# clairesonglee/HierarchicalGNN

Hardware: AMD Instinct MI355X
Metric: edges aggregated/sec on TrackML-1GeV graphs, latent=256 (higher is better)
Workload: dtype f32

## Files before the change

### hierarchicalgnn_amd/build.py

```python
from __future__ import annotations

import glob
import os
import shutil
import subprocess
import sys

HERE = os.path.dirname(os.path.abspath(__file__))
CSRC = os.path.join(HERE, "csrc")
OUT = os.path.join(CSRC, "libhgnn_hip.so")
ARCH = "gfx950"


def sources():
    return sorted(glob.glob(os.path.join(CSRC, "*.hip")))


def _deps():
    return sources() + sorted(glob.glob(os.path.join(CSRC, "*.h"))) + \
        [os.path.join(HERE, "..", "include", "hgnn_hip.h")]


def up_to_date() -> bool:
    if not os.path.exists(OUT):
        return False
    t = os.path.getmtime(OUT)
    return all(os.path.getmtime(p) <= t for p in _deps())


def build(force: bool = False, verbose: bool = True) -> str:
    if not force and up_to_date():
        return OUT
    hipcc = shutil.which("hipcc") or "/opt/rocm/bin/hipcc"
    if not os.path.exists(hipcc):
        raise RuntimeError("hipcc not found: cannot build libhgnn_hip.so")
    objs = []
    procs = []
    for src in sources():
        obj = src[:-4] + ".o"
        objs.append(obj)
        if not force and os.path.exists(obj) and all(
                os.path.getmtime(p) <= os.path.getmtime(obj)
                for p in [src] + [d for d in _deps() if d.endswith(".h")]):
            continue
        cmd = [hipcc, "-O3", "-std=c++17", f"--offload-arch={ARCH}", "-fPIC", "-c", src, "-o", obj]
        if verbose:
            print(" ".join(cmd), flush=True)
        procs.append((cmd, subprocess.Popen(cmd)))
    for cmd, p in procs:
        if p.wait() != 0:
            raise RuntimeError("build failed: " + " ".join(cmd))
    cmd = [hipcc, f"--offload-arch={ARCH}", "-shared", "-fPIC", "-o", OUT] + objs
    if verbose:
        print(" ".join(cmd), flush=True)
    subprocess.check_call(cmd)
    return OUT


if __name__ == "__main__":
    print(build(force="--force" in sys.argv))
```

### hierarchicalgnn_amd/csrc/capi.hip

```cpp
#include "common.h"
#include "options.h"
#include <climits>
#include <cstdlib>
#include <cstring>

namespace hgnn {
static thread_local char g_err[512] = "";

void set_error(const char* fmt, ...) {
    va_list ap;
    va_start(ap, fmt);
    vsnprintf(g_err, sizeof(g_err), fmt, ap);
    va_end(ap);
}

static const struct {
    const char* name;
    int* value;
    int lo, hi;
    const char* takes;
} kOptions[] = {
    {"nt_loads", &g_opt_nt_loads, INT_MIN, INT_MAX, nullptr},
    {"nt_stores", &g_opt_nt_stores, INT_MIN, INT_MAX, nullptr},
    {"k1_one_launch", &g_opt_k1_one_launch, 0, 1, "takes 0 or 1"},
    {"k1_item_order", &g_opt_k1_item_order, 0, 1, "takes 0 or 1"},
#ifdef HGNN_K1_SWEEP
    {"k1_window", &g_opt_k1_window, INT_MIN, INT_MAX, nullptr},
    {"k1_waves", &g_opt_k1_waves, INT_MIN, INT_MAX, nullptr},
#endif
    {"mlp_ablate", &g_opt_mlp_ablate, INT_MIN, INT_MAX, nullptr},
    {"mlp_split_variant", &g_opt_mlp_split_variant, INT_MIN, INT_MAX, nullptr},
    {"mlp_split3_rows128", &f3::g_opt_split3_rows128, 0, 2,
     "takes 0 or 1 (2 = experimental tile, needs HGNN_EXPERIMENTAL=1)"},
    {"mlp_split3_one_wg", &f3::g_opt_split3_one_wg, INT_MIN, INT_MAX, nullptr},
};
}

using namespace hgnn;

extern "C" int hgnn_abi_version(void) { return HGNN_ABI_VERSION; }
extern "C" const char* hgnn_last_error(void) { return hgnn::g_err; }
extern "C" int hgnn_sizeof_plan(void) { return (int)sizeof(hgnn_plan); }
extern "C" int hgnn_sizeof_mlp_desc(void) { return (int)sizeof(hgnn_mlp_desc); }

extern "C" int hgnn_set_option(const char* name, int value) {
    HGNN_REQUIRE(name != nullptr, "hgnn_set_option: name is NULL");
    for (const auto& o : kOptions) {
        if (strcmp(name, o.name)) continue;
        const bool experimental = o.value == &f3::g_opt_split3_rows128 && value == 2;
        if (value < o.lo || value > o.hi || (experimental && getenv("HGNN_EXPERIMENTAL") == nullptr)) {
            set_error("hgnn_set_option: %s %s", o.name, o.takes);
            return HGNN_ERR_INVALID_ARG;
        }
        *o.value = o.value == &g_opt_mlp_ablate ? value & 31 : value;
        return HGNN_OK;
    }
    set_error("hgnn_set_option: unknown option '%s'", name);
    return HGNN_ERR_INVALID_ARG;
}

extern "C" int hgnn_get_option(const char* name, int* value) {
    HGNN_REQUIRE(name != nullptr && value != nullptr, "hgnn_get_option: NULL pointer");
    for (const auto& o : kOptions) {
        if (strcmp(name, o.name)) continue;
        *value = *o.value;
        return HGNN_OK;
    }
    set_error("hgnn_get_option: unknown option '%s'", name);
    return HGNN_ERR_INVALID_ARG;
}
```

### hierarchicalgnn_amd/csrc/options.h

```cpp
#pragma once

namespace hgnn {

extern int g_opt_nt_loads;
extern int g_opt_nt_stores;
extern int g_opt_k1_one_launch;
extern int g_opt_k1_item_order;
#ifdef HGNN_K1_SWEEP
extern int g_opt_k1_window;
extern int g_opt_k1_waves;
#endif
extern int g_opt_mlp_ablate;
extern int g_opt_mlp_split_variant;
namespace f3 {
extern int g_opt_split3_rows128;
extern int g_opt_split3_one_wg;
}

}
```

### hierarchicalgnn_amd/csrc/rows_common.h

```cpp
#pragma once
#include "common.h"
#include "options.h"
#include <type_traits>

namespace hgnn {

typedef float f32x4 __attribute__((ext_vector_type(4)));

struct ItemView {
    const int32_t *begin, *end, *target;
    const int32_t* n_items;
    int64_t max_items;
    const int32_t *src_row, *perm, *wi_dst;
};

static inline ItemView work_items(const hgnn_plan* p) {
    return {p->wi_begin, p->wi_end, p->wi_target, p->counts + HGNN_CNT_WORK, p->max_work,
            p->src_row, p->perm, p->wi_dst};
}

static inline ItemView split_items(const hgnn_plan* p) {
    return {p->split_pbegin, p->split_pbegin + 1, p->split_dst, p->counts + HGNN_CNT_SPLIT, p->max_split,
            nullptr, nullptr, nullptr};
}

struct ItemExtra {
    const int32_t* order;
    int32_t* arrive;
    const int32_t *split_pbegin, *split_dst, *n_split;
    int32_t max_split;
};

static inline ItemExtra item_extra(const hgnn_plan* p, const int32_t* order, int32_t* arrive) {
    return {order, arrive, p->split_pbegin, p->split_dst, p->counts + HGNN_CNT_SPLIT, (int32_t)p->max_split};
}

template <int MAX_COLS, class Fn>
static inline void for_row_shape(int ncol, Fn&& fn) {
    using std::integral_constant;
    constexpr integral_constant<int, 1> one{};
    if (ncol <= 4) fn(integral_constant<int, 4>{}, one);
    else if (ncol <= 8) fn(integral_constant<int, 8>{}, one);
    else if (ncol <= 16) fn(integral_constant<int, 16>{}, one);
    else if (ncol <= 32) fn(integral_constant<int, 32>{}, one);
    else if (MAX_COLS <= 64 || ncol <= 64) fn(integral_constant<int, 64>{}, one);
    else if constexpr (MAX_COLS > 64) {
        if (ncol <= 128) fn(integral_constant<int, 64>{}, integral_constant<int, 2>{});
        else fn(integral_constant<int, 64>{}, integral_constant<int, 4>{});
    }
}

template <int WPB, class... P, class... A>
static inline void launch_items(void (*kernel)(P...), int64_t max_items, hipStream_t s, A... args) {
    const unsigned grid = (unsigned)ceil_div(max_items, WPB);
    if (grid) kernel<<<grid, WPB * 64, 0, s>>>(args...);
}

static inline unsigned capped_grid(int64_t blocks) {
    const int64_t cap = 256 * 8 * 4;
    return (unsigned)(blocks < 1 ? 1 : blocks > cap ? cap : blocks);
}
static inline unsigned stream_grid(int64_t n_tiles) { return capped_grid(ceil_div(n_tiles, kWavesPerBlock)); }

}
```

### hierarchicalgnn_amd/csrc/segreduce.hip

```cpp
#include "rows_common.h"

namespace hgnn {

int g_opt_nt_loads = 1;
int g_opt_nt_stores = 0;
int g_opt_k1_one_launch = 1;
int g_opt_k1_item_order = 0;

template <bool NT>
__device__ __forceinline__ f32x4 ld4(const void* p) {
    if constexpr (NT) return __builtin_nontemporal_load((const f32x4*)p);
    else return *(const f32x4*)p;
}

__device__ __forceinline__ bool last_chunk_arrives(const ItemExtra& x, int p, int lane, int& pbegin, int& nch,
                                                   int& dst) {
    int s = 0, hi = min(*x.n_split, x.max_split);
    while (hi - s > 1) {
        const int mid = (s + hi) >> 1;
        if (x.split_pbegin[mid] <= p) s = mid;
        else hi = mid;
    }
    pbegin = x.split_pbegin[s];
    nch = x.split_pbegin[s + 1] - pbegin;
    dst = x.split_dst[s];
    asm volatile("s_waitcnt vmcnt(0)" ::: "memory");
    __builtin_amdgcn_fence(__ATOMIC_RELEASE, "agent");
    asm volatile("s_waitcnt vmcnt(0)" ::: "memory");
    int seen = 0;
    if (lane == 0) seen = __hip_atomic_fetch_add(&x.arrive[s], 1, __ATOMIC_ACQ_REL, __HIP_MEMORY_SCOPE_AGENT);
    if (__builtin_amdgcn_readfirstlane(seen) != nch - 1) return false;
    asm volatile("s_waitcnt vmcnt(0)" ::: "memory");
    if (lane == 0) __hip_atomic_store(&x.arrive[s], 0, __ATOMIC_RELAXED, __HIP_MEMORY_SCOPE_AGENT);
    return true;
}

template <int RL, int VPL, int U, bool HAS_W, bool HAS_RS, bool NT, int TAG, int WPB, bool XCD>
__global__ __launch_bounds__(WPB * 64) void k_seg_reduce(
    const float* __restrict__ src, int F, int nvec, const int32_t* __restrict__ src_row,
    const int32_t* __restrict__ perm, const float* __restrict__ weight,
    const float* __restrict__ row_scale, const int32_t* __restrict__ wi_begin,
    const int32_t* __restrict__ wi_end, const int32_t* __restrict__ wi_target,
    const int32_t* __restrict__ n_items_ptr, int64_t max_items, float* __restrict__ out,
    float* __restrict__ partial, ItemExtra x) {
    constexpr int G = 64 / RL;
    const int lane = threadIdx.x & 63;
    int64_t bid = blockIdx.x;
    if (XCD) {
        const int64_t per_xcd = (gridDim.x + 7) / 8;
        bid = (bid % 8) * per_xcd + bid / 8;
    }
    int64_t item = bid * WPB + (threadIdx.x >> 6);
    const int n_items = *n_items_ptr;
    if (item >= max_items) return;
    if (x.order != nullptr) item = x.order[item];
    if (item >= n_items || item >= max_items) return;
    const int begin = __builtin_amdgcn_readfirstlane(wi_begin[item]);
    const int end = __builtin_amdgcn_readfirstlane(wi_end[item]);
    const int target = __builtin_amdgcn_readfirstlane(wi_target[item]);
    const int g = lane / RL;
    const int c = lane % RL;

    f32x4 acc[VPL];
#pragma unroll
    for (int v = 0; v < VPL; ++v) acc[v] = f32x4{0.f, 0.f, 0.f, 0.f};

    for (int base = begin; base < end; base += 64) {
        const int n = (end - base) < 64 ? (end - base) : 64;
        int my_row = 0;
        float my_w = 1.f;
        if (lane < n) {
            const int p = base + lane;
            my_row = src_row != nullptr ? src_row[p] : p;
            if (HAS_W) my_w = weight[perm != nullptr ? perm[p] : p];
            if (HAS_RS) my_w *= row_scale[my_row];
        }
        for (int j = 0; j < n; j += G * U) {
            f32x4 val[U][VPL];
            float w[U];
#pragma unroll
            for (int u = 0; u < U; ++u) {
                const int e = j + u * G + g;
                int r;
                if (G == 1) {
                    r = __builtin_amdgcn_readlane(my_row, (j + u) & 63);
                    w[u] = (HAS_W || HAS_RS)
                               ? __builtin_bit_cast(float, __builtin_amdgcn_readlane(
                                                               __builtin_bit_cast(int, my_w), (j + u) & 63))
                               : 1.f;
                } else {
                    r = __shfl(my_row, e & 63);
                    w[u] = (HAS_W || HAS_RS) ? __shfl(my_w, e & 63) : 1.f;
                }
                const bool ok = e < n;
                const float* rp = src + (size_t)r * (size_t)F;
#pragma unroll
                for (int v = 0; v < VPL; ++v) {
                    const int cv = c + v * 64;
                    if (ok && cv < nvec)
                        val[u][v] = ld4<NT>(rp + cv * 4);
                    else
                        val[u][v] = f32x4{0.f, 0.f, 0.f, 0.f};
                }
            }
#pragma unroll
            for (int u = 0; u < U; ++u) {
#pragma unroll
                for (int v = 0; v < VPL; ++v) {
                    if (HAS_W || HAS_RS)
                        acc[v] += val[u][v] * w[u];
                    else
                        acc[v] += val[u][v];
                }
            }
        }
    }
    if (G > 1) {
#pragma unroll
        for (int off = RL; off < 64; off <<= 1) {
#pragma unroll
            for (int v = 0; v < VPL; ++v) {
                acc[v].x += __shfl_xor(acc[v].x, off);
                acc[v].y += __shfl_xor(acc[v].y, off);
                acc[v].z += __shfl_xor(acc[v].z, off);
                acc[v].w += __shfl_xor(acc[v].w, off);
            }
        }
    }
    if (g == 0) {
        float* op = target >= 0 ? out + (size_t)target * (size_t)F
                                : partial + (size_t)(~target) * (size_t)F;
#pragma unroll
        for (int v = 0; v < VPL; ++v) {
            const int cv = c + v * 64;
            if (cv < nvec) *(f32x4*)(op + cv * 4) = acc[v];
        }
    }
    if constexpr (!HAS_W && !HAS_RS && TAG != 1) {
        if (x.arrive != nullptr && target < 0) {
            int pbegin, nch, dst;
            if (!last_chunk_arrives(x, ~target, lane, pbegin, nch, dst)) return;
#pragma unroll
            for (int v = 0; v < VPL; ++v) acc[v] = f32x4{0.f, 0.f, 0.f, 0.f};
            for (int k = g; k < nch; k += G) {
                const float* rp = partial + (size_t)(pbegin + k) * (size_t)F;
#pragma unroll
                for (int v = 0; v < VPL; ++v) {
                    const int cv = c + v * 64;
                    if (cv < nvec) acc[v] += ld4<NT>(rp + cv * 4);
                }
            }
            if (G > 1) {
#pragma unroll
                for (int off = RL; off < 64; off <<= 1) {
#pragma unroll
                    for (int v = 0; v < VPL; ++v) {
                        acc[v].x += __shfl_xor(acc[v].x, off);
                        acc[v].y += __shfl_xor(acc[v].y, off);
                        acc[v].z += __shfl_xor(acc[v].z, off);
                        acc[v].w += __shfl_xor(acc[v].w, off);
                    }
                }
            }
            float* op = out + (size_t)dst * (size_t)F;
#pragma unroll
            for (int v = 0; v < VPL; ++v) {
                const int cv = c + v * 64;
                if (g == 0 && cv < nvec) *(f32x4*)(op + cv * 4) = acc[v];
            }
        }
    }
}

template <int W, bool NT, int TAG, int WPB>
__global__ __launch_bounds__(WPB * 64) void k_seg_window(
    const float* __restrict__ src, int F, int nvec, const int32_t* __restrict__ src_row,
    const int32_t* __restrict__ wi_begin, const int32_t* __restrict__ wi_end,
    const int32_t* __restrict__ wi_target, const int32_t* __restrict__ n_items_ptr, int64_t max_items,
    float* __restrict__ out, float* __restrict__ partial, ItemExtra x) {
    static_assert(W >= 2 && 64 % W == 0, "a 64-row trip is a whole number of windows");
    constexpr bool IDENT = TAG != 0;
    const int lane = threadIdx.x & 63;
    int64_t item = (int64_t)blockIdx.x * WPB + __builtin_amdgcn_readfirstlane((int)(threadIdx.x >> 6));
    if (item >= max_items) return;
    if (x.order != nullptr) item = x.order[item];
    const bool valid = item < *n_items_ptr;
    item = item < max_items ? item : max_items - 1;
    const int begin = wi_begin[item];
    const int end = begin + (int)(((uint32_t)wi_end[item] - (uint32_t)begin) & (valid ? ~0u : 0u));
    const int target = wi_target[item];
    const uint32_t voff = (uint32_t)(lane < nvec ? lane : 0) * 16u;
    const size_t row_bytes = (size_t)F * sizeof(float);

    f32x4 acc = f32x4{0.f, 0.f, 0.f, 0.f};
    f32x4 ring[W];
    int ids = 0, ids_next = 0;
    if (!IDENT && begin < end) ids_next = src_row[min(begin + lane, end - 1)];
    for (int base = begin; base < end; base += 64) {
        const int n = min(end - base, 64);
        if (!IDENT) {
            ids = ids_next;
            if (base + 64 < end) ids_next = src_row[min(base + 64 + lane, end - 1)];
        }
        auto row = [&](int j) -> f32x4 {
            const uint32_t r = IDENT ? (uint32_t)(base + j) : (uint32_t)__builtin_amdgcn_readlane(ids, j);
            return ld4<NT>((const char*)src + (size_t)r * row_bytes + voff);
        };
        const int full = n & ~(W - 1), rem = n & (W - 1);
        const bool have = full > 0;
        if (have) {
#pragma unroll
            for (int u = 0; u < W; ++u) ring[u] = row(u);
        }
        for (int j = W; j < full; j += W) {
#pragma unroll
            for (int u = 0; u < W; ++u) {
                acc += ring[u];
                ring[u] = row(j + u);
                __builtin_amdgcn_sched_barrier(0);
            }
        }
        int j = full;
#pragma unroll
        for (int g = W / 2, o = 0; g >= 1; o += g, g >>= 1) {
            if (have) {
#pragma unroll
                for (int k = 0; k < g; ++k) acc += ring[o + k];
            }
            __builtin_amdgcn_sched_barrier(0);
            if (rem & g) {
#pragma unroll
                for (int k = 0; k < g; ++k) ring[o + k] = row(j + k);
                j += g;
            }
        }
        if (have) acc += ring[W - 1];
#pragma unroll
        for (int g = W / 2, o = 0; g >= 1; o += g, g >>= 1) {
            if (rem & g) {
#pragma unroll
                for (int k = 0; k < g; ++k) acc += ring[o + k];
            }
        }
    }
    float* op = target >= 0 ? out + (size_t)target * (size_t)F : partial + (size_t)(~target) * (size_t)F;
    if (valid && lane < nvec) *(f32x4*)(op + lane * 4) = acc;
    if constexpr (TAG != 1) {
        if (x.arrive != nullptr && valid && target < 0) {
            int pbegin, nch, dst;
            if (!last_chunk_arrives(x, ~target, lane, pbegin, nch, dst)) return;
            const char* pp = (const char*)partial + (size_t)pbegin * row_bytes + voff;
            acc = f32x4{0.f, 0.f, 0.f, 0.f};
#pragma unroll 1
            for (int k = 0; k < nch; k += 4) {
                f32x4 part[4];
#pragma unroll
                for (int u = 0; u < 4; ++u) part[u] = ld4<NT>(pp + (size_t)min(k + u, nch - 1) * row_bytes);
#pragma unroll
                for (int u = 0; u < 4; ++u) {
                    if (k + u < nch) acc += part[u];
                }
            }
            if (lane < nvec) *(f32x4*)(out + (size_t)dst * (size_t)F + lane * 4) = acc;
        }
    }
}

template <bool HAS_W, bool HAS_RS>
__global__ __launch_bounds__(256) void k_seg_reduce_scalar(
    const float* __restrict__ src, int F, const int32_t* __restrict__ src_row,
    const int32_t* __restrict__ perm, const float* __restrict__ weight,
    const float* __restrict__ row_scale, const int32_t* __restrict__ wi_begin,
    const int32_t* __restrict__ wi_end, const int32_t* __restrict__ wi_target,
    const int32_t* __restrict__ n_items_ptr, int64_t max_items, float* __restrict__ out,
    float* __restrict__ partial) {
    const int lane = threadIdx.x & 63;
    const int64_t item = (int64_t)blockIdx.x * kWavesPerBlock + (threadIdx.x >> 6);
    const int n_items = *n_items_ptr;
    if (item >= n_items || item >= max_items) return;
    const int begin = wi_begin[item], end = wi_end[item], target = wi_target[item];
    float* op = target >= 0 ? out + (size_t)target * (size_t)F : partial + (size_t)(~target) * (size_t)F;
    for (int col0 = 0; col0 < F; col0 += 64) {
        const int col = col0 + lane;
        float acc = 0.f;
        for (int p = begin; p < end; ++p) {
            const int r = src_row != nullptr ? src_row[p] : p;
            float w = 1.f;
            if (HAS_W) w = weight[perm != nullptr ? perm[p] : p];
            if (HAS_RS) w *= row_scale[r];
            if (col < F) acc += w * src[(size_t)r * (size_t)F + col];
        }
        if (col < F) op[col] = acc;
    }
}

template <int RL, int VPL, int U, bool HAS_W, bool HAS_RS>
__global__ __launch_bounds__(256) void k_gather_rows(const float* __restrict__ table, int F, int nvec,
                                                     const int32_t* __restrict__ idx, int64_t M,
                                                     const float* __restrict__ weight,
                                                     const float* __restrict__ row_scale,
                                                     float* __restrict__ out, bool nt_store) {
    constexpr int G = 64 / RL;
    const int lane = threadIdx.x & 63;
    const int g = lane / RL;
    const int c = lane % RL;
    const int64_t n_tiles = (M + 63) / 64;
    for (int64_t tile = (int64_t)blockIdx.x * kWavesPerBlock + (threadIdx.x >> 6); tile < n_tiles;
         tile += (int64_t)gridDim.x * kWavesPerBlock) {
        const int64_t base = tile * 64;
        const int n = (M - base) < 64 ? (int)(M - base) : 64;
        int my_idx = -1;
        float my_w = 1.f;
        if (lane < n) {
            my_idx = idx[base + lane];
            if (HAS_W) my_w = weight[base + lane];
            if (HAS_RS) my_w *= my_idx >= 0 ? row_scale[my_idx] : 0.f;
        }
        for (int j = 0; j < n; j += G * U) {
            f32x4 val[U][VPL];
            float w[U];
#pragma unroll
            for (int u = 0; u < U; ++u) {
                const int e = j + u * G + g;
                const int r = __shfl(my_idx, e & 63);
                w[u] = (HAS_W || HAS_RS) ? __shfl(my_w, e & 63) : 1.f;
                const bool ok = (e < n) && (r >= 0);
                const float* rp = table + (size_t)(ok ? r : 0) * (size_t)F;
#pragma unroll
                for (int v = 0; v < VPL; ++v) {
                    const int cv = c + v * 64;
                    if (ok && cv < nvec)
                        val[u][v] = *(const f32x4*)(rp + cv * 4);
                    else
                        val[u][v] = f32x4{0.f, 0.f, 0.f, 0.f};
                }
            }
#pragma unroll
            for (int u = 0; u < U; ++u) {
                const int e = j + u * G + g;
                if (e < n) {
                    float* op = out + (size_t)(base + e) * (size_t)F;
#pragma unroll
                    for (int v = 0; v < VPL; ++v) {
                        const int cv = c + v * 64;
                        if (cv < nvec) {
                            f32x4 x = (HAS_W || HAS_RS) ? val[u][v] * w[u] : val[u][v];
                            if (nt_store)
                                __builtin_nontemporal_store(x, (f32x4*)(op + cv * 4));
                            else
                                *(f32x4*)(op + cv * 4) = x;
                        }
                    }
                }
            }
        }
    }
}

template <int RL, int VPL, bool HAS_W, int WPB>
__global__ __launch_bounds__(WPB * 64) void k_spread_rows(
    const float* __restrict__ table, int F, int nvec, const int32_t* __restrict__ perm,
    const float* __restrict__ weight, const int32_t* __restrict__ wi_begin,
    const int32_t* __restrict__ wi_end, const int32_t* __restrict__ wi_dst,
    const int32_t* __restrict__ n_items_ptr, int64_t max_items, float* __restrict__ out, bool nt_store) {
    constexpr int G = 64 / RL;
    const int lane = threadIdx.x & 63;
    const int64_t item = (int64_t)blockIdx.x * WPB + (threadIdx.x >> 6);
    const int n_items = *n_items_ptr;
    if (item >= n_items || item >= max_items) return;
    const int begin = __builtin_amdgcn_readfirstlane(wi_begin[item]);
    const int end = __builtin_amdgcn_readfirstlane(wi_end[item]);
    if (begin >= end) return;
    const int dst = __builtin_amdgcn_readfirstlane(wi_dst[item]);
    const int g = lane / RL;
    const int c = lane % RL;
    f32x4 row[VPL];
    const float* rp = table + (size_t)dst * (size_t)F;
#pragma unroll
    for (int v = 0; v < VPL; ++v) {
        const int cv = c + v * 64;
        row[v] = cv < nvec ? *(const f32x4*)(rp + cv * 4) : f32x4{0.f, 0.f, 0.f, 0.f};
    }
    for (int base = begin; base < end; base += 64) {
        const int n = (end - base) < 64 ? (end - base) : 64;
        int my_e = 0;
        float my_w = 1.f;
        if (lane < n) {
            my_e = perm[base + lane];
            if (HAS_W) my_w = weight[my_e];
        }
        for (int j = 0; j < n; j += G) {
            const int k = j + g;
            const int e = __shfl(my_e, k & 63);
            const float w = HAS_W ? __shfl(my_w, k & 63) : 1.f;
            if (k < n) {
                float* op = out + (size_t)e * (size_t)F;
#pragma unroll
                for (int v = 0; v < VPL; ++v) {
                    const int cv = c + v * 64;
                    if (cv < nvec) {
                        const f32x4 x = HAS_W ? row[v] * w : row[v];
                        if (nt_store)
                            __builtin_nontemporal_store(x, (f32x4*)(op + cv * 4));
                        else
                            *(f32x4*)(op + cv * 4) = x;
                    }
                }
            }
        }
    }
}

template <bool HAS_W>
__global__ __launch_bounds__(256) void k_spread_rows_scalar(
    const float* __restrict__ table, int F, const int32_t* __restrict__ perm,
    const float* __restrict__ weight, const int32_t* __restrict__ wi_begin,
    const int32_t* __restrict__ wi_end, const int32_t* __restrict__ wi_dst,
    const int32_t* __restrict__ n_items_ptr, int64_t max_items, float* __restrict__ out) {
    const int lane = threadIdx.x & 63;
    const int64_t item = (int64_t)blockIdx.x * kWavesPerBlock + (threadIdx.x >> 6);
    const int n_items = *n_items_ptr;
    if (item >= n_items || item >= max_items) return;
    const int begin = wi_begin[item], end = wi_end[item], dst = wi_dst[item];
    for (int p = begin; p < end; ++p) {
        const int e = perm[p];
        const float w = HAS_W ? weight[e] : 1.f;
        for (int col = lane; col < F; col += 64)
            out[(size_t)e * F + col] = w * table[(size_t)dst * F + col];
    }
}

template <bool HAS_W, bool HAS_RS>
__global__ __launch_bounds__(256) void k_gather_rows_scalar(const float* __restrict__ table, int F,
                                                            const int32_t* __restrict__ idx, int64_t M,
                                                            const float* __restrict__ weight,
                                                            const float* __restrict__ row_scale,
                                                            float* __restrict__ out) {
    const int lane = threadIdx.x & 63;
    for (int64_t e = (int64_t)blockIdx.x * kWavesPerBlock + (threadIdx.x >> 6); e < M;
         e += (int64_t)gridDim.x * kWavesPerBlock) {
        const int r = idx[e];
        float w = 1.f;
        if (HAS_W) w = weight[e];
        if (HAS_RS) w *= r >= 0 ? row_scale[r] : 0.f;
        for (int col = lane; col < F; col += 64)
            out[(size_t)e * F + col] = r >= 0 ? w * table[(size_t)r * F + col] : 0.f;
    }
}

template <int RL, int VPL>
__global__ __launch_bounds__(256) void k_edge_dot(const float* __restrict__ A, const int32_t* __restrict__ ai,
                                                  const float* __restrict__ B, const int32_t* __restrict__ bi,
                                                  int F, int nvec, int64_t M, float* __restrict__ out) {
    constexpr int G = 64 / RL;
    const int lane = threadIdx.x & 63;
    const int g = lane / RL;
    const int c = lane % RL;
    const int64_t n_tiles = (M + 63) / 64;
    for (int64_t tile = (int64_t)blockIdx.x * kWavesPerBlock + (threadIdx.x >> 6); tile < n_tiles;
         tile += (int64_t)gridDim.x * kWavesPerBlock) {
        const int64_t base = tile * 64;
        const int n = (M - base) < 64 ? (int)(M - base) : 64;
        int my_a = -1, my_b = -1;
        if (lane < n) {
            my_a = ai != nullptr ? ai[base + lane] : (int)(base + lane);
            my_b = bi != nullptr ? bi[base + lane] : (int)(base + lane);
        }
        for (int j = 0; j < n; j += G * 2) {
            float s[2];
#pragma unroll
            for (int u = 0; u < 2; ++u) {
                const int e = j + u * G + g;
                const int ra = __shfl(my_a, e & 63);
                const int rb = __shfl(my_b, e & 63);
                const bool ok = (e < n) && ra >= 0 && rb >= 0;
                s[u] = 0.f;
                const float* pa = A + (size_t)(ok ? ra : 0) * (size_t)F;
                const float* pb = B + (size_t)(ok ? rb : 0) * (size_t)F;
#pragma unroll
                for (int v = 0; v < VPL; ++v) {
                    const int cv = c + v * 64;
                    if (ok && cv < nvec) {
                        f32x4 x = *(const f32x4*)(pa + cv * 4);
                        f32x4 y = *(const f32x4*)(pb + cv * 4);
                        s[u] += x.x * y.x + x.y * y.y + x.z * y.z + x.w * y.w;
                    }
                }
            }
#pragma unroll
            for (int u = 0; u < 2; ++u) {
                float t = s[u];
#pragma unroll
                for (int off = 1; off < RL; off <<= 1) t += __shfl_xor(t, off);
                const int e = j + u * G + g;
                if (c == 0 && e < n) out[base + e] = t;
            }
        }
    }
}

__global__ __launch_bounds__(256) void k_edge_dot_scalar(const float* __restrict__ A, const int32_t* __restrict__ ai,
                                                         const float* __restrict__ B, const int32_t* __restrict__ bi,
                                                         int F, int64_t M, float* __restrict__ out) {
    const int lane = threadIdx.x & 63;
    for (int64_t e = (int64_t)blockIdx.x * kWavesPerBlock + (threadIdx.x >> 6); e < M;
         e += (int64_t)gridDim.x * kWavesPerBlock) {
        const int ra = ai != nullptr ? ai[e] : (int)e;
        const int rb = bi != nullptr ? bi[e] : (int)e;
        float t = 0.f;
        if (ra >= 0 && rb >= 0)
            for (int col = lane; col < F; col += 64) t += A[(size_t)ra * F + col] * B[(size_t)rb * F + col];
#pragma unroll
        for (int off = 1; off < 64; off <<= 1) t += __shfl_xor(t, off);
        if (lane == 0) out[e] = t;
    }
}

struct SegArgs {
    const float* src;
    int F;
    const float* weight;
    const float* row_scale;
    float *out, *partial;
    ItemView items;
    ItemExtra extra;
};

template <int TAG, class Fn>
static void with_nt_loads(Fn&& fn) {
    if constexpr (TAG != 1) {
        if (g_opt_nt_loads) return fn(std::true_type{});
    }
    fn(std::false_type{});
}

template <int RL, int VPL, int U, bool W, bool RS, bool NT, int TAG, int WPB>
static void launch_seg3(const SegArgs& a, hipStream_t s) {
    const ItemView& v = a.items;
    launch_items<WPB>(k_seg_reduce<RL, VPL, U, W, RS, NT, TAG, WPB, false>, v.max_items, s, a.src, a.F, a.F / 4,
                      v.src_row, v.perm, a.weight, a.row_scale, v.begin, v.end, v.target, v.n_items, v.max_items,
                      a.out, a.partial, a.extra);
}

template <int RL, int VPL, int U, bool W, bool RS, int TAG>
static void launch_seg(const SegArgs& a, hipStream_t s) {
    with_nt_loads<TAG>([&](auto nt) { launch_seg3<RL, VPL, U, W, RS, decltype(nt)::value, TAG, 4>(a, s); });
}

template <int W, bool NT, int TAG, int WPB>
static void launch_window(const SegArgs& a, hipStream_t s) {
    const ItemView& v = a.items;
    launch_items<WPB>(k_seg_window<W, NT, TAG, WPB>, v.max_items, s, a.src, a.F, a.F / 4, v.src_row, v.begin, v.end,
                      v.target, v.n_items, v.max_items, a.out, a.partial, a.extra);
}

#ifdef HGNN_K1_SWEEP
int g_opt_k1_window = 16, g_opt_k1_waves = 8;
#endif

template <int TAG>
static void launch_seg_headline(const SegArgs& a, hipStream_t s) {
    with_nt_loads<TAG>([&](auto nt) {
        constexpr bool NT = decltype(nt)::value;
#ifdef HGNN_K1_SWEEP
        auto waves = [&](auto w) {
            constexpr int W = decltype(w)::value;
            if (g_opt_k1_waves == 4) launch_window<W, NT, TAG, 4>(a, s);
            else if (g_opt_k1_waves == 8) launch_window<W, NT, TAG, 8>(a, s);
            else launch_window<W, NT, TAG, 16>(a, s);
        };
        if (g_opt_k1_window == 0) launch_seg3<64, 1, 16, false, false, NT, TAG, 16>(a, s);
        else if (g_opt_k1_window == 8) waves(std::integral_constant<int, 8>{});
        else if (g_opt_k1_window == 32) waves(std::integral_constant<int, 32>{});
        else waves(std::integral_constant<int, 16>{});
#else
        launch_window<16, NT, TAG, 8>(a, s);
#endif
    });
}

constexpr int seg_rows_in_flight(int RL, int VPL) { return RL < 64 ? 4 : VPL == 1 ? 8 : VPL == 2 ? 4 : 2; }

template <bool W, bool RS, int TAG>
static void dispatch_seg(const SegArgs& a, hipStream_t s) {
    const ItemView& v = a.items;
    if (a.F % 4 != 0 || a.F > 1024)
        return launch_items<kWavesPerBlock>(k_seg_reduce_scalar<W, RS>, v.max_items, s, a.src, a.F, v.src_row, v.perm,
                                            a.weight, a.row_scale, v.begin, v.end, v.target, v.n_items, v.max_items,
                                            a.out, a.partial);
    for_row_shape<256>(a.F / 4, [&](auto rl, auto vpl) {
        constexpr int RL = decltype(rl)::value, VPL = decltype(vpl)::value;
        if constexpr (RL == 64 && VPL == 1 && !W && !RS) launch_seg_headline<TAG>(a, s);
        else launch_seg<RL, VPL, seg_rows_in_flight(RL, VPL), W, RS, TAG>(a, s);
    });
}

}

using namespace hgnn;

static int segment_reduce_f32(const char* who, const hgnn_plan* plan, const float* src, int32_t F,
                              const float* weight, const float* row_scale, float* out, float* partial,
                              int32_t* arrive, const int32_t* order, hipStream_t stream) {
    HGNN_REQUIRE(plan != nullptr, "%s: plan is NULL", who);
    HGNN_REQUIRE(F > 0, "%s: F must be positive (got %d)", who, F);
    if (plan->n_dst == 0) return HGNN_OK;
    HGNN_REQUIRE(out != nullptr, "%s: out is NULL", who);
    HGNN_REQUIRE(plan->n_rows == 0 || src != nullptr, "%s: src is NULL", who);
    HGNN_REQUIRE(plan->src_row != nullptr || !plan->has_gather,
                 "%s: src_row may only be NULL for a sorted plan without gather", who);
    HGNN_REQUIRE(partial != nullptr || plan->max_partial == 0, "%s: partial is NULL", who);
    HGNN_REQUIRE(((uintptr_t)src % 16 == 0 && (uintptr_t)out % 16 == 0 && (uintptr_t)partial % 16 == 0) || F % 4 != 0,
                 "%s: src/out/partial must be 16-byte aligned", who);
    SegArgs a = {src, F, weight, row_scale, out, partial, work_items(plan), ItemExtra{}};
    const bool plain_vec = !weight && !row_scale && F % 4 == 0 && F <= 1024;
    const bool one_launch = plain_vec && arrive != nullptr && g_opt_k1_one_launch;
    if (plain_vec) a.extra = item_extra(plan, g_opt_k1_item_order ? order : nullptr, one_launch ? arrive : nullptr);
    if (weight && row_scale) dispatch_seg<true, true, 0>(a, stream);
    else if (weight) dispatch_seg<true, false, 0>(a, stream);
    else if (row_scale) {
        set_error("%s: row_scale requires weight", who);
        return HGNN_ERR_UNSUPPORTED;
    } else if (plan->src_row == nullptr) {
        dispatch_seg<false, false, 2>(a, stream);
    } else dispatch_seg<false, false, 0>(a, stream);
    if (!one_launch)
        dispatch_seg<false, false, 1>(
            SegArgs{partial, F, nullptr, nullptr, out, partial, split_items(plan), ItemExtra{}}, stream);
    HGNN_CHECK_HIP(hipGetLastError());
    return HGNN_OK;
}

extern "C" int hgnn_segment_reduce_f32(const hgnn_plan* plan, const float* src, int32_t F,
                                       const float* weight, const float* row_scale, float* out,
                                       float* partial, hgnn_stream_t stream) {
    return segment_reduce_f32("hgnn_segment_reduce_f32", plan, src, F, weight, row_scale, out, partial, nullptr,
                              nullptr, (hipStream_t)stream);
}

extern "C" int hgnn_segment_reduce_f32_ex(const hgnn_plan* plan, const float* src, int32_t F,
                                          const float* weight, const float* row_scale, float* out,
                                          float* partial, int32_t* arrive, const int32_t* order,
                                          hgnn_stream_t stream) {
    HGNN_REQUIRE(plan == nullptr || arrive != nullptr, "hgnn_segment_reduce_f32_ex: arrive is NULL");
    return segment_reduce_f32("hgnn_segment_reduce_f32_ex", plan, src, F, weight, row_scale, out, partial, arrive,
                              order, (hipStream_t)stream);
}

constexpr int gather_rows_in_flight(int RL, int VPL) { return RL <= 8 ? 2 : RL < 64 ? 4 : VPL == 1 ? 8 : VPL == 2 ? 4 : 2; }

template <bool W, bool RS>
static void dispatch_gather(const float* table, int F, const int32_t* idx, int64_t M, const float* weight,
                            const float* row_scale, float* out, hipStream_t s) {
    if (F % 4 != 0 || F > 1024) {
        k_gather_rows_scalar<W, RS><<<stream_grid(M), kBlock, 0, s>>>(table, F, idx, M, weight, row_scale, out);
        return;
    }
    const unsigned grid = stream_grid(ceil_div(M, 64));
    const bool nt = g_opt_nt_stores != 0;
    for_row_shape<256>(F / 4, [&](auto rl, auto vpl) {
        constexpr int RL = decltype(rl)::value, VPL = decltype(vpl)::value;
        k_gather_rows<RL, VPL, gather_rows_in_flight(RL, VPL), W, RS><<<grid, kBlock, 0, s>>>(
            table, F, F / 4, idx, M, weight, row_scale, out, nt);
    });
}

extern "C" int hgnn_gather_rows_f32(const float* table, int64_t table_rows, int32_t F, const int32_t* idx,
                                    int64_t M, const float* weight, const float* row_scale, float* out,
                                    hgnn_stream_t stream_) {
    hipStream_t stream = (hipStream_t)stream_;
    HGNN_REQUIRE(F > 0 && M >= 0 && table_rows >= 0, "hgnn_gather_rows_f32: bad sizes");
    if (M == 0) return HGNN_OK;
    HGNN_REQUIRE(table != nullptr && idx != nullptr && out != nullptr, "hgnn_gather_rows_f32: NULL pointer");
    HGNN_REQUIRE(((uintptr_t)table % 16 == 0 && (uintptr_t)out % 16 == 0) || F % 4 != 0,
                 "hgnn_gather_rows_f32: table/out must be 16-byte aligned");
    if (weight && row_scale) dispatch_gather<true, true>(table, F, idx, M, weight, row_scale, out, stream);
    else if (weight) dispatch_gather<true, false>(table, F, idx, M, weight, row_scale, out, stream);
    else if (row_scale) dispatch_gather<false, true>(table, F, idx, M, weight, row_scale, out, stream);
    else dispatch_gather<false, false>(table, F, idx, M, weight, row_scale, out, stream);
    HGNN_CHECK_HIP(hipGetLastError());
    return HGNN_OK;
}

constexpr int spread_waves(int RL) { return RL < 64 ? 4 : 8; }

template <bool W>
static void dispatch_spread(const ItemView& v, const float* table, int F, const float* weight, float* out,
                            hipStream_t s) {
    if (F % 4 != 0 || F > 1024)
        return launch_items<kWavesPerBlock>(k_spread_rows_scalar<W>, v.max_items, s, table, F, v.perm, weight, v.begin,
                                            v.end, v.wi_dst, v.n_items, v.max_items, out);
    const bool nt = g_opt_nt_stores != 0;
    for_row_shape<256>(F / 4, [&](auto rl, auto vpl) {
        constexpr int RL = decltype(rl)::value, VPL = decltype(vpl)::value, WPB = spread_waves(RL);
        launch_items<WPB>(k_spread_rows<RL, VPL, W, WPB>, v.max_items, s, table, F, F / 4, v.perm, weight, v.begin,
                          v.end, v.wi_dst, v.n_items, v.max_items, out, nt);
    });
}

extern "C" int hgnn_spread_rows_f32(const hgnn_plan* plan, const float* table, int32_t F, const float* weight,
                                    float* out, hgnn_stream_t stream_) {
    hipStream_t stream = (hipStream_t)stream_;
    HGNN_REQUIRE(plan != nullptr, "hgnn_spread_rows_f32: plan is NULL");
    HGNN_REQUIRE(F > 0, "hgnn_spread_rows_f32: F must be positive");
    if (plan->n_rows == 0 || plan->n_dst == 0) return HGNN_OK;
    HGNN_REQUIRE(!plan->has_gather, "hgnn_spread_rows_f32: plan must be a plain destination plan");
    HGNN_REQUIRE(table != nullptr && out != nullptr, "hgnn_spread_rows_f32: NULL pointer");
    HGNN_REQUIRE(((uintptr_t)table % 16 == 0 && (uintptr_t)out % 16 == 0) || F % 4 != 0,
                 "hgnn_spread_rows_f32: table/out must be 16-byte aligned");
    if (weight) dispatch_spread<true>(work_items(plan), table, F, weight, out, stream);
    else dispatch_spread<false>(work_items(plan), table, F, weight, out, stream);
    HGNN_CHECK_HIP(hipGetLastError());
    return HGNN_OK;
}

extern "C" int hgnn_edge_dot_f32(const float* A, const int32_t* ai, int64_t a_rows, const float* B,
                                 const int32_t* bi, int64_t b_rows, int32_t F, int64_t M, float* out,
                                 hgnn_stream_t stream_) {
    hipStream_t stream = (hipStream_t)stream_;
    HGNN_REQUIRE(F > 0 && M >= 0, "hgnn_edge_dot_f32: bad sizes");
    if (M == 0) return HGNN_OK;
    HGNN_REQUIRE(A != nullptr && B != nullptr && out != nullptr, "hgnn_edge_dot_f32: NULL pointer");
    HGNN_REQUIRE((ai != nullptr || a_rows >= M) && (bi != nullptr || b_rows >= M),
                 "hgnn_edge_dot_f32: identity-indexed operand has fewer than M rows");
    if (F % 4 != 0 || F > 1024 || (uintptr_t)A % 16 != 0 || (uintptr_t)B % 16 != 0) {
        k_edge_dot_scalar<<<stream_grid(M), kBlock, 0, stream>>>(A, ai, B, bi, F, M, out);
    } else {
        const unsigned grid = stream_grid(ceil_div(M, 64));
        for_row_shape<256>(F / 4, [&](auto rl, auto vpl) {
            k_edge_dot<decltype(rl)::value, decltype(vpl)::value><<<grid, kBlock, 0, stream>>>(A, ai, B, bi, F, F / 4, M,
                                                                                              out);
        });
    }
    HGNN_CHECK_HIP(hipGetLastError());
    return HGNN_OK;
}
```

Baseline: 5.490 billion.

## Preload kernel args, reorder window kernel params, add cache-bypass output stores

Reorders k_seg_window's parameters so the item-lookup pointers come first, and compiles segreduce with kernarg preload so those arguments arrive in SGPRs before the first loads. A scheduling barrier and an asm use of the remaining scalar arguments push their loads behind the index fetches. It adds an option, on by default, that writes final output rows with sc0 sc1 global stores to bypass caches. It also turns the single-launch split-merge path off by default, so a second kernel launch handles the partial merge again, which costs extra launch overhead in exchange for removing the arrive/atomic tail.

```diff
diff --git a/hierarchicalgnn_amd/build.py b/hierarchicalgnn_amd/build.py
--- a/hierarchicalgnn_amd/build.py
+++ b/hierarchicalgnn_amd/build.py
@@ -10,6 +10,11 @@
 CSRC = os.path.join(HERE, "csrc")
 OUT = os.path.join(CSRC, "libhgnn_hip.so")
 ARCH = "gfx950"
+FILE_FLAGS = {"segreduce.hip": ["-mllvm", "-amdgpu-kernarg-preload-count=14"]}
+
+
+def compile_flags(src):
+    return ["-O3", "-std=c++17", f"--offload-arch={ARCH}", "-fPIC"] + FILE_FLAGS.get(os.path.basename(src), [])
 
 
 def sources():
@@ -43,7 +48,7 @@
                 os.path.getmtime(p) <= os.path.getmtime(obj)
                 for p in [src] + [d for d in _deps() if d.endswith(".h")]):
             continue
-        cmd = [hipcc, "-O3", "-std=c++17", f"--offload-arch={ARCH}", "-fPIC", "-c", src, "-o", obj]
+        cmd = [hipcc] + compile_flags(src) + ["-c", src, "-o", obj]
         if verbose:
             print(" ".join(cmd), flush=True)
         procs.append((cmd, subprocess.Popen(cmd)))
diff --git a/hierarchicalgnn_amd/csrc/capi.hip b/hierarchicalgnn_amd/csrc/capi.hip
--- a/hierarchicalgnn_amd/csrc/capi.hip
+++ b/hierarchicalgnn_amd/csrc/capi.hip
@@ -24,6 +24,7 @@
     {"nt_stores", &g_opt_nt_stores, INT_MIN, INT_MAX, nullptr},
     {"k1_one_launch", &g_opt_k1_one_launch, 0, 1, "takes 0 or 1"},
     {"k1_item_order", &g_opt_k1_item_order, 0, 1, "takes 0 or 1"},
+    {"k1_out_store", &g_opt_k1_out_store, 0, 1, "takes 0 or 1"},
 #ifdef HGNN_K1_SWEEP
     {"k1_window", &g_opt_k1_window, INT_MIN, INT_MAX, nullptr},
     {"k1_waves", &g_opt_k1_waves, INT_MIN, INT_MAX, nullptr},
diff --git a/hierarchicalgnn_amd/csrc/options.h b/hierarchicalgnn_amd/csrc/options.h
--- a/hierarchicalgnn_amd/csrc/options.h
+++ b/hierarchicalgnn_amd/csrc/options.h
@@ -6,6 +6,7 @@
 extern int g_opt_nt_stores;
 extern int g_opt_k1_one_launch;
 extern int g_opt_k1_item_order;
+extern int g_opt_k1_out_store;
 #ifdef HGNN_K1_SWEEP
 extern int g_opt_k1_window;
 extern int g_opt_k1_waves;
diff --git a/hierarchicalgnn_amd/csrc/rows_common.h b/hierarchicalgnn_amd/csrc/rows_common.h
--- a/hierarchicalgnn_amd/csrc/rows_common.h
+++ b/hierarchicalgnn_amd/csrc/rows_common.h
@@ -29,10 +29,12 @@
     int32_t* arrive;
     const int32_t *split_pbegin, *split_dst, *n_split;
     int32_t max_split;
+    int32_t out_store;
 };
 
-static inline ItemExtra item_extra(const hgnn_plan* p, const int32_t* order, int32_t* arrive) {
-    return {order, arrive, p->split_pbegin, p->split_dst, p->counts + HGNN_CNT_SPLIT, (int32_t)p->max_split};
+static inline ItemExtra item_extra(const hgnn_plan* p, const int32_t* order, int32_t* arrive, int out_store) {
+    return {order, arrive, p->split_pbegin, p->split_dst, p->counts + HGNN_CNT_SPLIT, (int32_t)p->max_split,
+            (int32_t)out_store};
 }
 
 template <int MAX_COLS, class Fn>
diff --git a/hierarchicalgnn_amd/csrc/segreduce.hip b/hierarchicalgnn_amd/csrc/segreduce.hip
--- a/hierarchicalgnn_amd/csrc/segreduce.hip
+++ b/hierarchicalgnn_amd/csrc/segreduce.hip
@@ -4,13 +4,19 @@
 
 int g_opt_nt_loads = 1;
 int g_opt_nt_stores = 0;
-int g_opt_k1_one_launch = 1;
+int g_opt_k1_one_launch = 0;
 int g_opt_k1_item_order = 0;
+int g_opt_k1_out_store = 1;
 
 template <bool NT>
 __device__ __forceinline__ f32x4 ld4(const void* p) {
     if constexpr (NT) return __builtin_nontemporal_load((const f32x4*)p);
     else return *(const f32x4*)p;
+}
+
+__device__ __forceinline__ void store_out_row(float* p, f32x4 v, int through) {
+    if (through) asm volatile("global_store_dwordx4 %0, %1, off sc0 sc1\n\ts_nop 1" : : "v"(p), "v"(v) : "memory");
+    else *(f32x4*)p = v;
 }
 
 __device__ __forceinline__ bool last_chunk_arrives(const ItemExtra& x, int p, int lane, int& pbegin, int& nch,
@@ -174,21 +180,27 @@
 
 template <int W, bool NT, int TAG, int WPB>
 __global__ __launch_bounds__(WPB * 64) void k_seg_window(
-    const float* __restrict__ src, int F, int nvec, const int32_t* __restrict__ src_row,
-    const int32_t* __restrict__ wi_begin, const int32_t* __restrict__ wi_end,
-    const int32_t* __restrict__ wi_target, const int32_t* __restrict__ n_items_ptr, int64_t max_items,
-    float* __restrict__ out, float* __restrict__ partial, ItemExtra x) {
+    const int32_t* __restrict__ order, const int32_t* __restrict__ n_items_ptr, const int32_t* __restrict__ wi_begin,
+    const int32_t* __restrict__ wi_end, const int32_t* __restrict__ wi_target, const int32_t* __restrict__ src_row,
+    int64_t max_items, const float* __restrict__ src, int F, int nvec, float* __restrict__ out,
+    float* __restrict__ partial, ItemExtra x) {
     static_assert(W >= 2 && 64 % W == 0, "a 64-row trip is a whole number of windows");
     constexpr bool IDENT = TAG != 0;
     const int lane = threadIdx.x & 63;
-    int64_t item = (int64_t)blockIdx.x * WPB + __builtin_amdgcn_readfirstlane((int)(threadIdx.x >> 6));
-    if (item >= max_items) return;
-    if (x.order != nullptr) item = x.order[item];
-    const bool valid = item < *n_items_ptr;
+    const int64_t slot = (int64_t)blockIdx.x * WPB + __builtin_amdgcn_readfirstlane((int)(threadIdx.x >> 6));
+    int64_t item = slot < max_items ? slot : max_items - 1;
+    if (order != nullptr) item = order[item];
+    const bool in_range = slot < max_items && item < max_items;
     item = item < max_items ? item : max_items - 1;
+    const int n_items = *n_items_ptr;
     const int begin = wi_begin[item];
-    const int end = begin + (int)(((uint32_t)wi_end[item] - (uint32_t)begin) & (valid ? ~0u : 0u));
+    const int end_raw = wi_end[item];
     const int target = wi_target[item];
+    __builtin_amdgcn_sched_barrier(0);
+    asm volatile("" : : "s"(src_row), "s"(src), "s"(F), "s"(nvec), "s"(out), "s"(partial), "s"(x.arrive),
+                 "s"(x.split_pbegin), "s"(x.split_dst), "s"(x.n_split), "s"(x.max_split), "s"(x.out_store));
+    const bool valid = in_range && item < n_items;
+    const int end = begin + (int)(((uint32_t)end_raw - (uint32_t)begin) & (valid ? ~0u : 0u));
     const uint32_t voff = (uint32_t)(lane < nvec ? lane : 0) * 16u;
     const size_t row_bytes = (size_t)F * sizeof(float);
 
@@ -244,7 +256,7 @@
         }
     }
     float* op = target >= 0 ? out + (size_t)target * (size_t)F : partial + (size_t)(~target) * (size_t)F;
-    if (valid && lane < nvec) *(f32x4*)(op + lane * 4) = acc;
+    if (valid && lane < nvec) store_out_row(op + lane * 4, acc, target >= 0 ? x.out_store : 0);
     if constexpr (TAG != 1) {
         if (x.arrive != nullptr && valid && target < 0) {
             int pbegin, nch, dst;
@@ -261,7 +273,7 @@
                     if (k + u < nch) acc += part[u];
                 }
             }
-            if (lane < nvec) *(f32x4*)(out + (size_t)dst * (size_t)F + lane * 4) = acc;
+            if (lane < nvec) store_out_row(out + (size_t)dst * (size_t)F + lane * 4, acc, x.out_store);
         }
     }
 }
@@ -550,8 +562,8 @@
 template <int W, bool NT, int TAG, int WPB>
 static void launch_window(const SegArgs& a, hipStream_t s) {
     const ItemView& v = a.items;
-    launch_items<WPB>(k_seg_window<W, NT, TAG, WPB>, v.max_items, s, a.src, a.F, a.F / 4, v.src_row, v.begin, v.end,
-                      v.target, v.n_items, v.max_items, a.out, a.partial, a.extra);
+    launch_items<WPB>(k_seg_window<W, NT, TAG, WPB>, v.max_items, s, a.extra.order, v.n_items, v.begin, v.end, v.target,
+                      v.src_row, v.max_items, a.src, a.F, a.F / 4, a.out, a.partial, a.extra);
 }
 
 #ifdef HGNN_K1_SWEEP
@@ -615,7 +627,9 @@
     SegArgs a = {src, F, weight, row_scale, out, partial, work_items(plan), ItemExtra{}};
     const bool plain_vec = !weight && !row_scale && F % 4 == 0 && F <= 1024;
     const bool one_launch = plain_vec && arrive != nullptr && g_opt_k1_one_launch;
-    if (plain_vec) a.extra = item_extra(plan, g_opt_k1_item_order ? order : nullptr, one_launch ? arrive : nullptr);
+    if (plain_vec)
+        a.extra = item_extra(plan, g_opt_k1_item_order ? order : nullptr, one_launch ? arrive : nullptr,
+                             g_opt_k1_out_store);
     if (weight && row_scale) dispatch_seg<true, true, 0>(a, stream);
     else if (weight) dispatch_seg<true, false, 0>(a, stream);
     else if (row_scale) {
```

Result: no change. 5.535 billion, median of 2 (+0.8%).
